# aanna0701/face-recognition-pytorch

Hardware: AMD Instinct MI355X
Metric: train imgs/sec IR-50-layout ResNet50 + ArcFace/PartialFC head, 112x112 (higher is better)
Workload: dtype bf16

## Files before the change

### face-recognition-pytorch_amd/frhip/csrc/igemm_nt.hip

```cpp
#include "igemm_nt.h"
#include "frhip.h"

namespace frhip {

bool halo_applicable(int dtype, int h, int w, int c, int k, int r, int s, int stride, int pad);
int halo_stat_rows(int dtype, int m, int w, int c, int k, int sign);
bool halo_xf_applicable(int dtype, int h, int w, int c, int k, int r, int s, int stride, int pad);
bool halo_lean_applies(int dtype, int n, int h, int w, int c, int k, int sign);
int halo_run(int dtype, const void* a, const void* b, void* out, const void* res, float* stats, const EpiBnRed& br,
             int n, int h, int w, int c, int k, int sign, hipStream_t stream, const float* xf_scale = nullptr,
             const float* xf_shift = nullptr, void* xf_out = nullptr);

enum { EPI_STORE = 0, EPI_ATOMIC = 1, EPI_SLAB = 2, EPI_LEAN = 3 };
extern int g_epi_lean;

template <typename T, int WM, int WN, int MT, int EPI>
__device__ __forceinline__ void nt_tile(const NtGeom& g, const void* __restrict__ a, const void* __restrict__ b, void* __restrict__ out,
                                        const void* __restrict__ res, float* __restrict__ stats, const EpiBnRed& br, int ntiles,
                                        uint32_t t, uint32_t total, char* smem) {
    typedef NtTile<T, WM, WN, MT> Tile;
    constexpr int WROWS = Tile::WROWS, THREADS = Tile::THREADS;
    const uint32_t lin = xcd_remap(t, total);
    const int ntile = (int)(lin % (uint32_t)ntiles), mtile = (int)(lin / (uint32_t)ntiles);
    const int ks_begin = blockIdx.y * g.ksteps_per_split;
    const int ks_end = min(g.ksteps, ks_begin + g.ksteps_per_split);

    NtMainloop<T, WM, WN, MT> ml;
    ml.run(g, a, b, smem, mtile, ntile, ks_begin, ks_end);

    const int lane = lane_id(), wave = wave_id();
    const int wm = wave / WN, wn = wave % WN;
    const int m0 = mtile * Tile::BM + wm * WROWS, n0 = ntile * Tile::BN + wn * 64;

    if constexpr (EPI == EPI_LEAN) {
        if (stats && br.y && !br.gelu_bwd) {
            constexpr int P = Tile::template stage_pitch<T>();
            float accs[2][4] = {{0.f, 0.f, 0.f, 0.f}, {0.f, 0.f, 0.f, 0.f}};
#pragma unroll
            for (int half = 0; half < 2; ++half) {
                EpiOperands<T, 64> eo;
                eo.fetch_fast(res, br.y, g.M, g.Nout, m0 + 64 * half, n0);
                const char* mine = ml.stage_half(smem, half);
                nt_epilogue_store_fast<T, WM, WN, 64, THREADS, Tile::BN>(mine, P, smem, g.M, g.Nout, out, res != nullptr, stats, br, eo, mtile, ntile,
                                                                         64 * P, accs);
            }
            epi_stats_tail_mfma<WM, WN, THREADS, Tile::BN>(accs[0], accs[1], smem, g.Nout, stats, mtile, ntile);
        } else {
            const char* mine = ml.template stage_out<T>(smem);
            nt_epilogue_store_lean<WM, WN, WROWS, THREADS, Tile::BN>(mine, Tile::template stage_pitch<T>(), smem, g.M, g.Nout, out, res, stats, br,
                                                                     mtile, ntile, m0, n0);
        }
    } else if constexpr (EPI == EPI_STORE) {
        EpiOperands<T, WROWS> eo;
        eo.fetch(res, (stats || br.gelu_bwd) ? br.y : nullptr, g.M, g.Nout, m0, n0, br.res_h, br.res_w, &br.map);
        const char* mine = ml.template stage_out<T>(smem);
        nt_epilogue_store<T, WM, WN, WROWS, THREADS, Tile::BN>(mine, Tile::template stage_pitch<T>(), smem, g.M, g.Nout, out,
                                                               res != nullptr, stats, br, eo, mtile, ntile, m0, n0);
    } else {
        constexpr int P = Tile::template stage_pitch<float>();
        const char* mine = ml.template stage_out<float>(smem);
        float* o = reinterpret_cast<float*>(out);
        const int n = n0 + lane;
        if constexpr (EPI == EPI_SLAB) o += (size_t)blockIdx.y * g.M * g.Nout;
        for (int row = 0; row < WROWS; ++row) {
            const int m = m0 + row;
            if (m < g.M && n < g.Nout) {
                const float v = *reinterpret_cast<const float*>(mine + row * P + lane * 4);
                if constexpr (EPI == EPI_SLAB) o[(size_t)m * g.Nout + n] = v;
                else atomicAdd(o + (size_t)m * g.Nout + n, v);
            }
        }
    }
}

template <typename T, int WM, int WN, int MT, int EPI>
__global__ __launch_bounds__(64 * WM * WN, (WM * WN) / 4) void nt_kernel(NtGeom g, const void* __restrict__ a,
                                                           const void* __restrict__ b, void* __restrict__ out,
                                                           const void* __restrict__ res, float* __restrict__ stats,
                                                           EpiBnRed br, int mtiles, int ntiles) {
    extern __shared__ __attribute__((aligned(16))) char smem[];
    const uint32_t total = (uint32_t)(mtiles * ntiles);
    if constexpr (EPI == EPI_LEAN) {
        for (uint32_t t = blockIdx.x; t < total; t += gridDim.x) {
            nt_tile<T, WM, WN, MT, EPI>(g, a, b, out, res, stats, br, ntiles, t, total, smem);
            if (t + gridDim.x < total) {
                asm volatile("s_waitcnt lgkmcnt(0)" ::: "memory");
                __builtin_amdgcn_s_barrier();
            }
        }
    } else {
        nt_tile<T, WM, WN, MT, EPI>(g, a, b, out, res, stats, br, ntiles, blockIdx.x, total, smem);
    }
}

template <typename T, int WM, int WN, int MT, int EPI>
static int nt_launch_cfg(const NtGeom& g, const void* a, const void* b, void* out, const void* res,
                         float* stats, const EpiBnRed& br, int splits, hipStream_t stream) {
    typedef NtTile<T, WM, WN, MT> Tile;
    const int mtiles = (g.M + Tile::BM - 1) / Tile::BM, ntiles = (g.Nout + Tile::BN - 1) / Tile::BN;
    const int lds = (EPI == EPI_STORE || EPI == EPI_LEAN) ? Tile::template lds_bytes<T>() : Tile::template lds_bytes<float>();
    auto kern = nt_kernel<T, WM, WN, MT, EPI>;
    if (set_dynamic_lds(reinterpret_cast<const void*>(kern), lds, "igemm_nt")) return FRHIP_ELAUNCH;
    dim3 grid(mtiles * ntiles, splits);
    if (EPI == EPI_LEAN) {
        const unsigned wgs = (unsigned)device_cu_count() & ~7u;
        if (wgs >= 8 && grid.x > wgs) grid.x = wgs;
    }
    hipLaunchKernelGGL(kern, grid, dim3(Tile::THREADS), lds, stream, g, a, b, out, res, stats, br, mtiles, ntiles);
    return check_launch("igemm_nt");
}

static int g_nt_tile = 0;

static int nt_pick_tile(int dtype, const NtGeom& g) {
    if (g_nt_tile) return (dtype != FRHIP_DT_BF16 && g_nt_tile >= 3) ? 1 : g_nt_tile;
    if ((g.Nout % 128) != 0 && g.Nout <= 256) return 2;
    if (dtype == FRHIP_DT_BF16 && (g.Nout % 256) == 0 && g.M >= 256 * 64) return 4;
    return 1;
}

static const EpiBnRed NO_BNRED = {nullptr, nullptr, nullptr, nullptr, nullptr, 0, 0, {0, 0, 0, 0, 0, 0}, nullptr, nullptr, 0};

static int nt_dispatch(int dtype, const NtGeom& g, const void* a, const void* b, void* out, const void* res,
                       float* stats, const EpiBnRed& br, int splits, bool atomic, hipStream_t stream) {
    const int tile = nt_pick_tile(dtype, g);
#define NT_GO(T, WM, WN, MT)                                                                              \
    return atomic ? nt_launch_cfg<T, WM, WN, MT, EPI_ATOMIC>(g, a, b, out, res, stats, br, splits, stream)     \
                  : nt_launch_cfg<T, WM, WN, MT, EPI_STORE>(g, a, b, out, res, stats, br, splits, stream)
    if (dtype == FRHIP_DT_BF16 && (tile == 3 || tile == 4)) {
        if (tile == 4 && !atomic && splits == 1 && g_epi_lean && nt_lean_ok(true, g.M, g.Nout, br, stats))
            return nt_launch_cfg<bf16_t, 2, 4, 8, EPI_LEAN>(g, a, b, out, res, stats, br, splits, stream);
        if (tile == 4 && !atomic) return nt_launch_cfg<bf16_t, 2, 4, 8, EPI_STORE>(g, a, b, out, res, stats, br, splits, stream);
        NT_GO(bf16_t, 4, 2, 4);
    }
    return by_dtype(dtype, "igemm_nt", [&](auto t) {
        typedef decltype(t) T;
        if (tile == 2) NT_GO(T, 4, 1, 4);
        NT_GO(T, 2, 2, 4);
    });
#undef NT_GO
}

static int esize(int dtype) { return dtype == FRHIP_DT_BF16 ? 2 : 4; }

static int fill_geom(NtGeom& g, int dtype, int n, int h, int w, int c, int ho, int wo, int k, int r, int s,
                     int stride, int pad, int mode, const char* who) {
    const int bke = NT_ROWB / esize(dtype);
    if (n <= 0 || h <= 0 || w <= 0 || c <= 0 || k <= 0 || (c % bke) != 0 || (k % 8) != 0 || (stride != 1 && stride != 2)) {
        set_error("%s: unsupported shape n=%d h=%d w=%d c=%d k=%d stride=%d (c must be a multiple of %d, k of 8)",
                  who, n, h, w, c, k, stride, bke);
        return FRHIP_EINVAL;
    }
    const long long a_bytes = 1LL * n * h * w * c * esize(dtype), b_bytes = 1LL * k * r * s * c * esize(dtype);
    if (a_bytes > 0x7fffffffLL || b_bytes > 0x7fffffffLL || 1LL * n * ho * wo > 0x7fffffffLL) {
        set_error("%s: tensor exceeds the 2 GiB buffer-addressing window", who);
        return FRHIP_EINVAL;
    }
    g.H = h; g.W = w; g.C = c; g.Ho = ho; g.Wo = wo; g.R = r; g.S = s; g.stride = stride; g.pad = pad; g.mode = mode;
    g.M = n * ho * wo; g.Nout = k; g.Ktot = r * s * c;
    g.ksteps = r * s * (c / bke); g.ksteps_per_split = g.ksteps;
    g.a_bytes = (uint32_t)a_bytes; g.b_bytes = (uint32_t)b_bytes;
    g.par_a = -1; g.par_b = -1; g.hc = 0; g.wc = 0; g.par_r0 = 0; g.par_s0 = 0;
    return FRHIP_OK;
}

static bool dgrad_by_parity(const NtGeom& g) { return g.mode == 1 && g.stride == 2 && g.R == 3 && g.S == 3 && g.pad == 1; }

static int nt_block_rows(int dtype, const NtGeom& g) {
    static const int bm_of[5] = {128, 128, 256, 256, 256};
    return bm_of[nt_pick_tile(dtype, g)];
}

static int parity_class(const NtGeom& g, int dtype, int a, int b, NtGeom& gc, OutMap& map) {
    gc = g;
    gc.par_a = a; gc.par_b = b;
    gc.hc = (g.Ho - a + 1) / 2; gc.wc = (g.Wo - b + 1) / 2;
    gc.par_r0 = (a + g.pad) & 1; gc.par_s0 = (b + g.pad) & 1;
    const int nr = (g.R - gc.par_r0 + 1) / 2, ns = (g.S - gc.par_s0 + 1) / 2;
    const int n_img = g.M / (g.Ho * g.Wo);
    gc.M = n_img * gc.hc * gc.wc;
    gc.ksteps = nr * ns * (g.C / (NT_ROWB / (dtype == FRHIP_DT_BF16 ? 2 : 4)));
    gc.ksteps_per_split = gc.ksteps;
    map.hc = gc.hc; map.wc = gc.wc; map.ho = g.Ho; map.wo = g.Wo; map.a = a; map.b = b;
    return gc.M;
}

}

using namespace frhip;

extern "C" int frhip_nt_block_m(int nout) {
    return ((nout % 128) == 0 || nout > 256) ? 128 : 256;
}
extern "C" int frhip_conv_stat_rows(int dtype, int m, int k, int h, int w, int c, int r, int s, int stride, int pad) {
    if (halo_applicable(dtype, h, w, c, k, r, s, stride, pad)) return halo_stat_rows(dtype, m, w, c, k, +1);
    NtGeom g; g.M = m; g.Nout = k;
    static const int bm_of[5] = {128, 128, 256, 256, 256};
    const int bm = bm_of[nt_pick_tile(dtype, g)];
    return (m + bm - 1) / bm;
}
extern "C" int frhip_set_nt_tile(int tile) { const int old = g_nt_tile; g_nt_tile = tile; return old; }

extern "C" int frhip_conv_fwd(int dtype, const void* x, const void* w, void* y, float* stats_partial,
                              int n, int h, int wd, int c, int k, int r, int s, int stride, int pad,
                              hipStream_t stream) {
    if (const int rc = by_dtype(dtype, "frhip_conv_fwd", [](auto) { return FRHIP_OK; })) return rc;
    NtGeom g;
    const int ho = (h + 2 * pad - r) / stride + 1, wo = (wd + 2 * pad - s) / stride + 1;
    int rc = fill_geom(g, dtype, n, h, wd, c, ho, wo, k, r, s, stride, pad, 0, "frhip_conv_fwd");
    if (rc) return rc;
    if (halo_applicable(dtype, h, wd, c, k, r, s, stride, pad))
        return halo_run(dtype, x, w, y, nullptr, stats_partial, NO_BNRED, n, h, wd, c, k, +1, stream);
    return nt_dispatch(dtype, g, x, w, y, nullptr, stats_partial, NO_BNRED, 1, false, stream);
}

extern "C" int frhip_conv_fwd_affine(int dtype, const void* x, const void* w, void* y, const float* scale, const float* shift, int relu,
                                     const void* residual, int n, int h, int wd, int c, int k, int r, int s, int stride, int pad,
                                     hipStream_t stream) {
    if (const int rc = by_dtype(dtype, "frhip_conv_fwd_affine", [](auto) { return FRHIP_OK; })) return rc;
    if (!scale || !shift) { set_error("frhip_conv_fwd_affine: scale and shift are required"); return FRHIP_EINVAL; }
    NtGeom g;
    const int ho = (h + 2 * pad - r) / stride + 1, wo = (wd + 2 * pad - s) / stride + 1;
    int rc = fill_geom(g, dtype, n, h, wd, c, ho, wo, k, r, s, stride, pad, 0, "frhip_conv_fwd_affine");
    if (rc) return rc;
    if (halo_applicable(dtype, h, wd, c, k, r, s, stride, pad) && halo_lean_applies(dtype, n, h, wd, c, k, +1)) {
        EpiBnRed br = NO_BNRED;
        br.aff_scale = scale; br.aff_shift = shift; br.aff_relu = relu;
        return halo_run(dtype, x, w, y, residual, nullptr, br, n, h, wd, c, k, +1, stream);
    }
    rc = frhip_conv_fwd(dtype, x, w, y, nullptr, n, h, wd, c, k, r, s, stride, pad, stream);
    if (rc) return rc;
    return frhip_bn_apply(dtype, y, scale, shift, residual, nullptr, nullptr, relu, y, n * ho * wo, k, stream);
}

extern "C" int frhip_conv_bnrelu_fusable(int dtype, int h, int wd, int c, int k, int r, int s, int stride, int pad) {
    return halo_xf_applicable(dtype, h, wd, c, k, r, s, stride, pad) ? 1 : 0;
}

extern "C" int frhip_conv_fwd_bnrelu(int dtype, const void* x, const float* in_scale, const float* in_shift, const void* w, void* y,
                                     float* stats_partial, void* act_out, int n, int h, int wd, int c, int k, int r, int s, int stride,
                                     int pad, hipStream_t stream) {
    if (const int rc = by_dtype(dtype, "frhip_conv_fwd_bnrelu", [](auto) { return FRHIP_OK; })) return rc;
    if (!in_scale || !in_shift || !halo_xf_applicable(dtype, h, wd, c, k, r, s, stride, pad)) {
        set_error("frhip_conv_fwd_bnrelu: not fusable for this shape (ask frhip_conv_bnrelu_fusable first)");
        return FRHIP_EINVAL;
    }
    return halo_run(dtype, x, w, y, nullptr, stats_partial, NO_BNRED, n, h, wd, c, k, +1, stream, in_scale, in_shift, act_out);
}

static int dgrad_run(int dtype, const void* dy, const void* wt, void* dx, const void* residual, float* stats,
                     const EpiBnRed& br, int n, int h, int wd, int c, int k, int r, int s, int stride, int pad,
                     hipStream_t stream, const char* who) {
    NtGeom g;
    const int ho = (h + 2 * pad - r) / stride + 1, wo = (wd + 2 * pad - s) / stride + 1;
    int rc = fill_geom(g, dtype, n, ho, wo, k, h, wd, c, r, s, stride, pad, 1, who);
    if (rc) return rc;
    if (halo_applicable(dtype, h, wd, k, c, r, s, stride, pad))
        return halo_run(dtype, dy, wt, dx, residual, stats, br, n, h, wd, k, c, -1, stream);
    if (dgrad_by_parity(g)) {
        float* st = stats;
        for (int cls = 0; cls < 4; ++cls) {
            NtGeom gc; EpiBnRed bc = br;
            if (parity_class(g, dtype, cls >> 1, cls & 1, gc, bc.map) == 0) continue;
            rc = nt_dispatch(dtype, gc, dy, wt, dx, residual, st, bc, 1, false, stream);
            if (rc) return rc;
            if (st) st += (size_t)((gc.M + nt_block_rows(dtype, gc) - 1) / nt_block_rows(dtype, gc)) * 2 * gc.Nout;
        }
        return FRHIP_OK;
    }
    return nt_dispatch(dtype, g, dy, wt, dx, residual, stats, br, 1, false, stream);
}

extern "C" int frhip_conv_dgrad(int dtype, const void* dy, const void* wt, void* dx, const void* residual,
                                int n, int h, int wd, int c, int k, int r, int s, int stride, int pad,
                                hipStream_t stream) {
    if (const int rc = by_dtype(dtype, "frhip_conv_dgrad", [](auto) { return FRHIP_OK; })) return rc;
    return dgrad_run(dtype, dy, wt, dx, residual, nullptr, NO_BNRED, n, h, wd, c, k, r, s, stride, pad, stream, "frhip_conv_dgrad");
}

extern "C" int frhip_dgrad_stat_rows(int dtype, int n, int h, int wd, int c, int k, int r, int s, int stride, int pad) {
    const int m = n * h * wd;
    if (halo_applicable(dtype, h, wd, k, c, r, s, stride, pad)) return halo_stat_rows(dtype, m, wd, k, c, -1);
    NtGeom g; g.M = m; g.Nout = c;
    g.mode = 1; g.stride = stride; g.R = r; g.S = s; g.pad = pad; g.Ho = h; g.Wo = wd; g.C = k;
    if (dgrad_by_parity(g)) {
        int rows = 0;
        for (int cls = 0; cls < 4; ++cls) {
            NtGeom gc; OutMap map;
            const int mc = parity_class(g, dtype, cls >> 1, cls & 1, gc, map);
            rows += (mc + nt_block_rows(dtype, gc) - 1) / nt_block_rows(dtype, gc);
        }
        return rows;
    }
    const int bm = nt_block_rows(dtype, g);
    return (m + bm - 1) / bm;
}

extern "C" int frhip_conv_dgrad_fused(int dtype, const void* dy, const void* wt, void* dx, const void* residual,
                                      int residual_stride, const void* y_bn, const float* mean, const float* invstd,
                                      const float* mask_scale, const float* mask_shift, float* stats_partial, int n, int h,
                                      int wd, int c, int k, int r, int s, int stride, int pad, hipStream_t stream) {
    if (const int rc = by_dtype(dtype, "frhip_conv_dgrad_fused", [](auto) { return FRHIP_OK; })) return rc;
    if (residual_stride != 1 && residual_stride != 2) { set_error("frhip_conv_dgrad_fused: residual_stride must be 1 or 2"); return FRHIP_EINVAL; }
    if (y_bn && (!mean || !invstd || !stats_partial || (mask_scale && !mask_shift))) {
        set_error("frhip_conv_dgrad_fused: y_bn needs mean, invstd and stats_partial");
        return FRHIP_EINVAL;
    }
    EpiBnRed br = {y_bn, mean, invstd, mask_scale, mask_shift, 0, 0, {0, 0, 0, 0, 0, 0}, nullptr, nullptr, 0};
    if (residual && residual_stride == 2) { br.res_h = h; br.res_w = wd; }
    return dgrad_run(dtype, dy, wt, dx, residual, y_bn ? stats_partial : nullptr, br, n, h, wd, c, k, r, s, stride, pad, stream,
                     "frhip_conv_dgrad_fused");
}

extern "C" int frhip_conv_dgrad_fused_rs(int dtype, const void* dy, const void* wt, void* dx, const void* residual,
                                         int residual_stride, const void* y_bn, const float* mean, const float* invstd,
                                         const float* mask_scale, const float* mask_shift, const float* rowscale, int rows_per,
                                         float keep_scale, float* stats_partial, int n, int h, int wd, int c, int k, int r, int s,
                                         int stride, int pad, hipStream_t stream) {
    if (const int rc = by_dtype(dtype, "frhip_conv_dgrad_fused_rs", [](auto) { return FRHIP_OK; })) return rc;
    if (residual_stride != 1 && residual_stride != 2) { set_error("frhip_conv_dgrad_fused_rs: residual_stride must be 1 or 2"); return FRHIP_EINVAL; }
    if (!y_bn || !mean || !invstd || !stats_partial || (mask_scale && !mask_shift) || !rowscale || rows_per <= 0 ||
        (long long)n * h * wd % rows_per != 0) {
        set_error("frhip_conv_dgrad_fused_rs: y_bn, mean, invstd, stats_partial, rowscale and a rows_per that divides the rows are required");
        return FRHIP_EINVAL;
    }
    EpiBnRed br = {y_bn, mean, invstd, mask_scale, mask_shift, 0, 0, {0, 0, 0, 0, 0, 0}, nullptr, nullptr, 0};
    br.rowkeep = rowscale; br.rows_per = rows_per; br.keep_scale = keep_scale;
    if (residual && residual_stride == 2) { br.res_h = h; br.res_w = wd; }
    return dgrad_run(dtype, dy, wt, dx, residual, stats_partial, br, n, h, wd, c, k, r, s, stride, pad, stream, "frhip_conv_dgrad_fused_rs");
}

extern "C" int frhip_conv_dgrad_bnred(int dtype, const void* dy, const void* wt, void* dx, const void* residual,
                                      const void* y_bn, const float* mean, const float* invstd, const float* mask_scale,
                                      const float* mask_shift, float* stats_partial, int n, int h, int wd, int c, int k,
                                      int r, int s, int stride, int pad, hipStream_t stream) {
    if (const int rc = by_dtype(dtype, "frhip_conv_dgrad_bnred", [](auto) { return FRHIP_OK; })) return rc;
    if (!y_bn || !mean || !invstd || !stats_partial || (mask_scale && !mask_shift)) {
        set_error("frhip_conv_dgrad_bnred: y_bn, mean, invstd and stats_partial are required");
        return FRHIP_EINVAL;
    }
    return frhip_conv_dgrad_fused(dtype, dy, wt, dx, residual, 1, y_bn, mean, invstd, mask_scale, mask_shift, stats_partial,
                                  n, h, wd, c, k, r, s, stride, pad, stream);
}

extern "C" int frhip_linear_fwd(int dtype, const void* a, const void* w, const float* bias, void* out, void* act_out,
                                float* stats_partial, int m, int n, int k, hipStream_t stream) {
    if (const int rc = by_dtype(dtype, "frhip_linear_fwd", [](auto) { return FRHIP_OK; })) return rc;
    NtGeom g;
    int rc = fill_geom(g, dtype, m, 1, 1, k, 1, 1, n, 1, 1, 1, 0, 0, "frhip_linear_fwd");
    if (rc) return rc;
    EpiBnRed br = NO_BNRED;
    br.bias = bias; br.act = act_out;
    return nt_dispatch(dtype, g, a, w, out, nullptr, stats_partial, br, 1, false, stream);
}

extern "C" int frhip_linear_dgrad_gelu(int dtype, const void* dy, const void* wt, const void* pre, void* dx,
                                       float* stats_partial, int m, int n, int k, hipStream_t stream) {
    if (const int rc = by_dtype(dtype, "frhip_linear_dgrad_gelu", [](auto) { return FRHIP_OK; })) return rc;
    if (!pre) { set_error("frhip_linear_dgrad_gelu: the saved pre-activation is required"); return FRHIP_EINVAL; }
    NtGeom g;
    int rc = fill_geom(g, dtype, m, 1, 1, k, 1, 1, n, 1, 1, 1, 0, 0, "frhip_linear_dgrad_gelu");
    if (rc) return rc;
    EpiBnRed br = NO_BNRED;
    br.y = pre; br.gelu_bwd = 1;
    return nt_dispatch(dtype, g, dy, wt, dx, nullptr, stats_partial, br, 1, false, stream);
}

namespace frhip {
__global__ __launch_bounds__(256) void nt_slab_reduce_kernel(const float* __restrict__ slabs, int splits, size_t elems,
                                                             const float* __restrict__ bias, int n, float* __restrict__ out) {
    const size_t i = ((size_t)blockIdx.x * 256 + threadIdx.x) * 4;
    if (i >= elems) return;
    f32x4_t acc = *reinterpret_cast<const f32x4_t*>(slabs + i);
    for (int s = 1; s < splits; ++s) acc += *reinterpret_cast<const f32x4_t*>(slabs + (size_t)s * elems + i);
    if (bias) acc += *reinterpret_cast<const f32x4_t*>(bias + (i % (size_t)n));
    *reinterpret_cast<f32x4_t*>(out + i) = acc;
}
}

extern "C" int frhip_gemm_nt_splitk(int dtype, const void* a, const void* b, const float* bias, float* out, int m, int n,
                                    int k, int splits, float* slabs, size_t slab_bytes, hipStream_t stream) {
    return by_dtype(dtype, "frhip_gemm_nt_splitk", [&](auto t) {
        NtGeom g;
        int rc = fill_geom(g, dtype, m, 1, 1, k, 1, 1, n, 1, 1, 1, 0, 0, "frhip_gemm_nt_splitk");
        if (rc) return rc;
        if (n % 4) { set_error("frhip_gemm_nt_splitk: n must be a multiple of 4"); return FRHIP_EINVAL; }
        if (splits < 1) splits = 1;
        if (splits > g.ksteps) splits = g.ksteps;
        g.ksteps_per_split = (g.ksteps + splits - 1) / splits;
        splits = (g.ksteps + g.ksteps_per_split - 1) / g.ksteps_per_split;
        const size_t elems = (size_t)m * n;
        if (!slabs || slab_bytes < elems * 4 * (size_t)splits) { set_error("frhip_gemm_nt_splitk: workspace too small (%zu bytes needed)", elems * 4 * (size_t)splits); return FRHIP_EINVAL; }
        rc = nt_launch_cfg<decltype(t), 2, 2, 4, EPI_SLAB>(g, a, b, slabs, nullptr, nullptr, NO_BNRED, splits, stream);
        if (rc) return rc;
        hipLaunchKernelGGL(nt_slab_reduce_kernel, dim3((unsigned)((elems / 4 + 255) / 256)), dim3(256), 0, stream, slabs, splits, elems, bias, n, out);
        return check_launch("frhip_gemm_nt_splitk/reduce");
    });
}

extern "C" int frhip_gemm_nt(int dtype, const void* a, const void* b, void* out, int m, int n, int k,
                             int splits, int atomic_f32, hipStream_t stream) {
    if (const int rc = by_dtype(dtype, "frhip_gemm_nt", [](auto) { return FRHIP_OK; })) return rc;
    NtGeom g;
    int rc = fill_geom(g, dtype, m, 1, 1, k, 1, 1, n, 1, 1, 1, 0, 0, "frhip_gemm_nt");
    if (rc) return rc;
    if (!atomic_f32 || splits < 1) splits = 1;
    if (splits > g.ksteps) splits = g.ksteps;
    g.ksteps_per_split = (g.ksteps + splits - 1) / splits;
    splits = (g.ksteps + g.ksteps_per_split - 1) / g.ksteps_per_split;
    return nt_dispatch(dtype, g, a, b, out, nullptr, nullptr, NO_BNRED, splits, atomic_f32 != 0, stream);
}
```

### include/frhip.h

```cpp
#ifndef FRHIP_H
#define FRHIP_H
#include <stddef.h>
#include <stdint.h>

#ifdef __cplusplus
extern "C" {
#endif

#ifndef FRHIP_STREAM_T
#define FRHIP_STREAM_T
#ifdef __HIP_PLATFORM_AMD__
#include <hip/hip_runtime_api.h>
typedef hipStream_t frhip_stream_t;
#else
typedef void* frhip_stream_t;
#endif
#endif

#define FRHIP_OK 0
#define FRHIP_EINVAL (-1)
#define FRHIP_ELAUNCH (-2)
#define FRHIP_DT_BF16 0
#define FRHIP_DT_F32 1

const char* frhip_last_error(void);
int frhip_abi_version(void);
int frhip_spin(long long ticks, frhip_stream_t stream);

int frhip_nt_block_m(int k);
int frhip_conv_stat_rows(int dtype, int m, int k, int h, int w, int c, int r, int s, int stride, int pad);
int frhip_set_wgrad_taps9(int enabled);
int frhip_set_conv_halo(int enabled);
int frhip_set_halo_wide_dirs(int dirs);
int frhip_set_epi_lean(int enabled);
int frhip_set_ew_batch(int enabled);
int frhip_set_nt_tile(int tile);
int frhip_conv_fwd_affine(int dtype, const void* x, const void* w, void* y, const float* scale, const float* shift, int relu,
                          const void* residual, int n, int h, int wd, int c, int k, int r, int s, int stride, int pad,
                          frhip_stream_t stream);
int frhip_conv_fwd(int dtype, const void* x, const void* w, void* y, float* stats_partial,
                   int n, int h, int wd, int c, int k, int r, int s, int stride, int pad, frhip_stream_t stream);
int frhip_conv_dgrad(int dtype, const void* dy, const void* wt, void* dx, const void* residual,
                     int n, int h, int wd, int c, int k, int r, int s, int stride, int pad, frhip_stream_t stream);
int frhip_dgrad_stat_rows(int dtype, int n, int h, int wd, int c, int k, int r, int s, int stride, int pad);
int frhip_conv_dgrad_bnred(int dtype, const void* dy, const void* wt, void* dx, const void* residual,
                           const void* y_bn, const float* mean, const float* invstd, const float* mask_scale,
                           const float* mask_shift, float* stats_partial, int n, int h, int wd, int c, int k,
                           int r, int s, int stride, int pad, frhip_stream_t stream);
int frhip_conv_dgrad_fused(int dtype, const void* dy, const void* wt, void* dx, const void* residual, int residual_stride,
                           const void* y_bn, const float* mean, const float* invstd, const float* mask_scale,
                           const float* mask_shift, float* stats_partial, int n, int h, int wd, int c, int k,
                           int r, int s, int stride, int pad, frhip_stream_t stream);
int frhip_conv_dgrad_fused_rs(int dtype, const void* dy, const void* wt, void* dx, const void* residual, int residual_stride,
                              const void* y_bn, const float* mean, const float* invstd, const float* mask_scale,
                              const float* mask_shift, const float* rowscale, int rows_per, float keep_scale,
                              float* stats_partial, int n, int h, int wd, int c, int k, int r, int s, int stride, int pad,
                              frhip_stream_t stream);
int frhip_conv_wgrad(int dtype, const void* dy, const void* x, float* dw, int n, int h, int w, int c,
                     int k, int r, int s, int stride, int pad, int splits, float* workspace, size_t workspace_bytes,
                     frhip_stream_t stream);
int frhip_conv_wgrad_chain_ok(int dtype, int n, int h, int w, int c, int k, int r, int s, int stride, int pad);
int frhip_conv_wgrad_chain(int dtype, const void* dy, const void* x, int n, int h, int w, int c, int k, float* slabs,
                           size_t slab_bytes, float* prev_dw, const float* prev_slabs, int prev_k, int prev_c, int prev_splits,
                           int* splits_out, frhip_stream_t stream);
int frhip_conv_wgrad_chain_finish(float* dw, float* slabs, int k, int c, int splits, frhip_stream_t stream);
int frhip_wgrad_plan(int dtype, int n, int h, int w, int c, int kc, int ldp, int r, int s, int stride, int pad, int splits,
                     int have_workspace, size_t workspace_bytes, int overwrite, int transform, int* plan_out);
int frhip_linear_fwd(int dtype, const void* a, const void* w, const float* bias, void* out, void* act_out,
                     float* stats_partial, int m, int n, int k, frhip_stream_t stream);
int frhip_linear_dgrad_gelu(int dtype, const void* dy, const void* wt, const void* pre, void* dx, float* stats_partial,
                            int m, int n, int k, frhip_stream_t stream);
int frhip_gemm_nt(int dtype, const void* a, const void* b, void* out, int m, int n, int k, int splits,
                  int atomic_f32, frhip_stream_t stream);
int frhip_gemm_nt_splitk(int dtype, const void* a, const void* b, const float* bias, float* out, int m, int n, int k,
                         int splits, float* slabs, size_t slab_bytes, frhip_stream_t stream);
int frhip_gemm_tn(int dtype, const void* p, const void* q, float* out, int m, int kc, int ldp, int c,
                  int splits, float* workspace, size_t workspace_bytes, frhip_stream_t stream);
int frhip_gemm_tn_overwrite(int dtype, const void* p, const void* q, float* out, int m, int kc, int ldp, int c,
                            float* workspace, size_t workspace_bytes, frhip_stream_t stream);

int frhip_colreduce_blocks(int rows, int c, int dtype);
int frhip_colstats(int dtype, const void* x, int rows, int c, float* partial, frhip_stream_t stream);
int frhip_bn_finalize(const float* partial, int nparts, float* scratch, int c, float count,
                      const float* gamma, const float* beta, float* running_mean, float* running_var,
                      float momentum, float eps, float* mean, float* invstd, float* scale, float* shift,
                      frhip_stream_t stream);
int frhip_bn_eval_affine(int c, const float* gamma, const float* beta, const float* running_mean,
                         const float* running_var, float eps, float* scale, float* shift, frhip_stream_t stream);
int frhip_bn_standin_state(int c, const float* gamma, const float* beta, float k, float* mean, float* invstd, float* scale,
                           float* shift, frhip_stream_t stream);
int frhip_bn_apply(int dtype, const void* y, const float* scale, const float* shift, const void* res,
                   const float* res_scale, const float* res_shift, int relu, void* out, int rows, int c,
                   frhip_stream_t stream);
int frhip_bn_bwd_reduce(int dtype, const void* dout, const void* y, const float* mean, const float* invstd,
                        const float* mask_scale, const float* mask_shift, int rows, int c, float* partial,
                        frhip_stream_t stream);
int frhip_bn_bwd_finalize(const float* partial, int nparts, float* scratch, int c, float count,
                          const float* gamma, const float* mean, const float* invstd, float* dgamma,
                          float* dbeta, float* ca, float* cb, float* cc, frhip_stream_t stream);
int frhip_bn_eval_state(int c, const float* gamma, const float* beta, const float* running_mean, const float* running_var, float eps,
                        float* mean, float* invstd, float* scale, float* shift, frhip_stream_t stream);
int frhip_bn_bwd_finalize_eval(const float* partial, int nparts, float* scratch, int c, float count,
                               const float* gamma, const float* mean, const float* invstd, float* dgamma,
                               float* dbeta, float* ca, float* cb, float* cc, frhip_stream_t stream);
int frhip_bn_bwd_apply(int dtype, const void* dout, const void* y, const float* ca, const float* cb,
                       const float* cc, const float* mask_scale, const float* mask_shift, void* dy,
                       int rows, int c, frhip_stream_t stream);
int frhip_bn_apply_rs(int dtype, const void* y, const float* scale, const float* shift, const void* res, const float* rowscale,
                      int rows_per, void* out, int rows, int c, frhip_stream_t stream);
int frhip_bn_bwd_reduce_rs(int dtype, const void* dout, const void* y, const float* mean, const float* invstd, const float* rowscale,
                           int rows_per, int rows, int c, float* partial, frhip_stream_t stream);
int frhip_bn_bwd_apply_rs(int dtype, const void* dout, const void* y, const float* ca, const float* cb, const float* cc,
                          const float* rowscale, int rows_per, void* dy, int rows, int c, frhip_stream_t stream);
int frhip_sum_partials(const float* partial, int nparts, int c, int which, float* out_accum, frhip_stream_t stream);
int frhip_add_bias(float* x, const float* bias, int rows, int c, frhip_stream_t stream);
int frhip_cast_from_f32(int dtype, const float* src, void* dst, size_t n, frhip_stream_t stream);
int frhip_cast_to_f32(int dtype, const void* src, float* dst, size_t n, frhip_stream_t stream);

int frhip_stem_im2col(int dtype, const float* x, void* col, int b, int h, int w, int stride, frhip_stream_t stream);
int frhip_bn_relu_maxpool_fwd(int dtype, const void* y, const float* scale, const float* shift, void* out,
                              uint8_t* argmax, int b, int h, int w, int c, frhip_stream_t stream);
int frhip_maxpool_bwd(int dtype, const void* dpool, const uint8_t* argmax, void* da, int b, int h, int w,
                      int c, frhip_stream_t stream);

int frhip_pack_wt(int dtype, const float* w, void* wt, int k, int rs, int c, frhip_stream_t stream);
int frhip_transpose2d(int dtype_in, int dtype_out, const void* in, void* out, int rows, int cols, int ld_out,
                      frhip_stream_t stream);
int frhip_pack_stem(int dtype, const float* w, void* wp, int k, int kin, int kp, frhip_stream_t stream);
int frhip_unpack_stem_grad(const float* dwp, float* dw, int k, int kin, int kp, frhip_stream_t stream);
int frhip_fc_permute(int dtype, const float* w, void* wp, int nout, int c, int hw, frhip_stream_t stream);
int frhip_fc_unpermute_grad(const float* dwp, float* dw, int nout, int c, int hw, frhip_stream_t stream);
int frhip_pfc_sample_max_local(void);
int frhip_pfc_sample(const int64_t* labels, int n, long long class_start, int num_local, const float* u, int num_sample,
                     int64_t* index_out, int* rel_out, int64_t* n_positive, frhip_stream_t stream);
int frhip_gather_rows(const float* src, const int64_t* index, float* dst, int n, int d, frhip_stream_t stream);
int frhip_scatter_rows(const float* src, const int64_t* index, float* dst, int n, int d, frhip_stream_t stream);

int frhip_head_dw_ok(int dtype, int n, int classes, int d);
int frhip_head_dw(int dtype, const void* dt, int ldt, const void* ehat, const void* what, const float* wnorm, float* dw,
                  int n, int classes, int d, float out_scale, frhip_stream_t stream);
int frhip_l2norm_rows(int dtype, const float* x, void* xhat, float* norms, int rows, int d, float eps,
                      frhip_stream_t stream);
int frhip_l2norm_bwd(int dtype, const float* dxhat, const void* xhat, const float* norms, float* dx,
                     int rows, int d, float out_scale, frhip_stream_t stream);
int frhip_l2norm_bwd_norm(int dtype, const float* dxhat, const void* xhat, const float* norms, const float* dnorm, float* dx,
                          int rows, int d, float out_scale, frhip_stream_t stream);
int frhip_head_groups(int num_classes);
int frhip_head_fwd(int dtype, const void* ehat, const void* what, const int* labels, int n, int classes,
                   int d, float s, float m, float* part_max, float* part_sum, float* ztarget,
                   float* rowmax, float* rowsum, frhip_stream_t stream);
int frhip_head_rescale(float* rowsum, const float* local_max, const float* global_max, int n, frhip_stream_t stream);
int frhip_head_target_prob(const float* ztarget, const int* labels, const float* rowmax, const float* rowsum,
                           float* q, int n, frhip_stream_t stream);
int frhip_head_pack_stats(const float* ztarget, const int* labels, const float* rowmax, const float* rowsum,
                          float* packed, int n, frhip_stream_t stream);
int frhip_head_merge_stats(const float* gathered, int world_size, int n, float* rowmax, float* rowsum, float* q,
                           frhip_stream_t stream);
int frhip_head_loss(const float* q, int n, float* loss, frhip_stream_t stream);
int frhip_head_bwd_dt(int dtype, const void* ehat, const void* what, const int* labels, int n, int classes,
                      int d, float s, float m, const float* rowmax, const float* rowsum, float gscale,
                      const float* upstream, void* dt, int ldt, void* dtt, int ldtt, frhip_stream_t stream);

#define FRHIP_MARGIN_ARCFACE 0
#define FRHIP_MARGIN_COSFACE 1
typedef struct { int kind; int easy; float s, m, filter_thr; } frhip_margin_t;
int frhip_head_fwd_ex(int dtype, const void* ehat, const void* what, const int* labels, int n, int classes,
                      int d, const frhip_margin_t* margin, float* part_max, float* part_sum, float* ztarget,
                      float* rowmax, float* rowsum, frhip_stream_t stream);
int frhip_head_bwd_dt_ex(int dtype, const void* ehat, const void* what, const int* labels, int n, int classes,
                         int d, const frhip_margin_t* margin, const float* rowmax, const float* rowsum, float gscale,
                         const float* upstream, void* dt, int ldt, void* dtt, int ldtt, frhip_stream_t stream);

typedef struct { float s, eps; const float* m_ang; const float* m_add; } frhip_margin_rows_t;
int frhip_adaface_margins(const float* norms, int n, double m, double h, double t_alpha, double eps, int update, float* batch_mean,
                          float* batch_std, float* m_ang, float* m_add, frhip_stream_t stream);
int frhip_magface_margins(const float* norms, int n, double l_a, double u_a, double l_m, double u_m, float* m_ang, float* m_add,
                          float* reg, frhip_stream_t stream);
int frhip_magface_norm_grad(const float* norms, const float* packed, int world_size, int n, const float* rowmax, const float* rowsum,
                            float s, float eps, double l_a, double u_a, double l_m, double u_m, double lambda_g, double gscale,
                            const float* upstream, double out_scale, float* dnorm, frhip_stream_t stream);
int frhip_head_fwd_rows(int dtype, const void* ehat, const void* what, const int* labels, int n, int classes,
                        int d, const frhip_margin_rows_t* margin, float* part_max, float* part_sum, float* ztarget,
                        float* rowmax, float* rowsum, frhip_stream_t stream);
int frhip_head_bwd_dt_rows(int dtype, const void* ehat, const void* what, const int* labels, int n, int classes,
                           int d, const frhip_margin_rows_t* margin, const float* rowmax, const float* rowsum, float gscale,
                           const float* upstream, void* dt, int ldt, void* dtt, int ldtt, frhip_stream_t stream);

int frhip_head_sub_max(void);
int frhip_head_fwd_sub(int dtype, const void* ehat, const void* what, const int* labels, int n, int classes, int d,
                       int subcenters, const frhip_margin_t* margin, float* part_max, float* part_sum, float* ztarget,
                       int* tsub, float* rowmax, float* rowsum, frhip_stream_t stream);
int frhip_head_fwd_sub_rows(int dtype, const void* ehat, const void* what, const int* labels, int n, int classes, int d,
                            int subcenters, const frhip_margin_rows_t* margin, float* part_max, float* part_sum,
                            float* ztarget, int* tsub, float* rowmax, float* rowsum, frhip_stream_t stream);
int frhip_head_bwd_dt_sub(int dtype, const void* ehat, const void* what, const int* labels, int n, int classes, int d,
                          int subcenters, const frhip_margin_t* margin, const float* rowmax, const float* rowsum,
                          float gscale, const float* upstream, void* dt, int ldt, int ldp, void* dtt, int ldtt,
                          frhip_stream_t stream);
int frhip_head_bwd_dt_sub_rows(int dtype, const void* ehat, const void* what, const int* labels, int n, int classes, int d,
                               int subcenters, const frhip_margin_rows_t* margin, const float* rowmax, const float* rowsum,
                               float gscale, const float* upstream, void* dt, int ldt, int ldp, void* dtt, int ldtt,
                               frhip_stream_t stream);

int frhip_conv_bnrelu_fusable(int dtype, int h, int wd, int c, int k, int r, int s, int stride, int pad);
int frhip_conv_fwd_bnrelu(int dtype, const void* x, const float* in_scale, const float* in_shift, const void* w, void* y,
                          float* stats_partial, void* act_out, int n, int h, int wd, int c, int k, int r, int s, int stride,
                          int pad, frhip_stream_t stream);
int frhip_conv_wgrad_bnrelu_fusable(int dtype, int n, int h, int w, int c, int k, int r, int s, int stride, int pad);
int frhip_conv_wgrad_bnrelu(int dtype, const void* dy, const void* x, const float* in_scale, const float* in_shift,
                            float* dw, int n, int h, int w, int c, int k, int r, int s, int stride, int pad, int splits,
                            float* workspace, size_t workspace_bytes, frhip_stream_t stream);

int frhip_quant_fp8_weights(const float* w, void* w8, float* scale, int k, int rowlen, frhip_stream_t stream);
typedef struct { const float* w; void* w8; float* scale; int32_t k, rowlen, row_begin, pad_; } frhip_q8w;
int frhip_quant_fp8_weights_multi(const frhip_q8w* table, int ntensors, int nrows, frhip_stream_t stream);
int frhip_fp8_saturation(int op);
int frhip_quant_fp8(int dtype, const void* x, void* x8, size_t n, float inv_scale, frhip_stream_t stream);
int frhip_bn_apply_q8(int dtype, const void* y, const float* scale, const float* shift, const void* res,
                      const float* res_scale, const float* res_shift, int relu, void* out, void* out8, float inv_q,
                      int rows, int c, frhip_stream_t stream);
int frhip_conv_fwd_fp8(const void* x8, const void* w8, const float* wscale, float act_scale, void* y,
                       float* stats_partial, int n, int h, int wd, int c, int k, int r, int s, int stride, int pad,
                       frhip_stream_t stream);
int frhip_fp8_stat_rows(int m, int k);
int frhip_fp8_conv_stat_rows(int m, int k, int h, int w, int c, int r, int s, int stride, int pad);
int frhip_set_fp8_halo(int enabled);
int frhip_linear_fwd_fp8(const void* a8, const void* w8, const float* wscale, float act_scale, const float* bias,
                         void* out, float* stats_partial, int m, int n, int k, frhip_stream_t stream);

typedef struct frhip_cpb_block {
    const void* coords;
    const void* index;
    const void* w0;
    const void* b0;
    const void* w2;
    const void* logit_scale;
    void* bias;
    void* scale;
    const void* dbias;
    const void* dscale;
    void* dw0;
    void* db0;
    void* dw2;
    void* dlogit_scale;
    int entries, tokens, heads, pad_;
} frhip_cpb_block;
int frhip_cpb_limits(int* max_entries, int* max_heads, int* hidden);
int frhip_cpb_scratch_floats(int nblocks);
int frhip_cpb_fwd(const frhip_cpb_block* blocks_dev, int nblocks, float* scratch, frhip_stream_t stream);
int frhip_cpb_bwd(const frhip_cpb_block* blocks_dev, int nblocks, float* scratch, frhip_stream_t stream);

int frhip_margin_fwd(float* logits, const int64_t* labels, int n, int c, float s, float m, int kind, float* tsave,
                     frhip_stream_t stream);
int frhip_margin_bwd(const float* gout, const int64_t* labels, const float* tsave, int n, int c, float s, float m,
                     int kind, float* gin, frhip_stream_t stream);
int frhip_margin_fwd_ex(float* logits, const int64_t* labels, int n, int c, const frhip_margin_t* margin, float* tsave,
                        uint64_t* filtered, frhip_stream_t stream);
int frhip_margin_bwd_ex(const float* gout, const int64_t* labels, const float* tsave, const uint64_t* filtered, int n, int c,
                        const frhip_margin_t* margin, float* gin, frhip_stream_t stream);
int frhip_margin_fwd_rows(const float* logits, const int64_t* labels, int n, int c, const frhip_margin_rows_t* margin, float* out,
                          frhip_stream_t stream);
int frhip_margin_bwd_rows(const float* gout, const float* logits, const int64_t* labels, int n, int c,
                          const frhip_margin_rows_t* margin, float* gin, frhip_stream_t stream);
int frhip_rows_max(const float* x, int n, int c, float* rowmax, frhip_stream_t stream);
int frhip_rows_exp_sum(float* x, int n, int c, const float* rowmax, float* rowsum, frhip_stream_t stream);
int frhip_rows_normalize(float* x, int n, int c, const float* rowsum, const int64_t* labels, float* ptarget,
                         frhip_stream_t stream);
int frhip_ce_grad(float* p, int n, int c, const int64_t* labels, float inv_n, const float* upstream,
                  frhip_stream_t stream);

int frhip_winattn_fwd(int dtype, const void* qkv, const float* bias, const float* scale, void* out, int b, int h,
                      int w, int c, int heads, int ws, int shift, frhip_stream_t stream);
int frhip_winattn_bwd(int dtype, const void* qkv, const void* dout, const float* bias, const float* scale,
                      void* dqkv, float* dbias, float* dscale, int b, int h, int w, int c, int heads,
                      int ws, int shift, float* workspace, size_t workspace_bytes, frhip_stream_t stream);
int frhip_winattn_bwd_colsum(int dtype, const void* qkv, const void* dout, const float* bias, const float* scale,
                             void* dqkv, float* dbias, float* dscale, float* dqkv_colsum, int b, int h, int w, int c,
                             int heads, int ws, int shift, float* workspace, size_t workspace_bytes, frhip_stream_t stream);
int frhip_winattn_bwd_qvbias(int dtype, const void* qkv, const void* dout, const float* bias, const float* scale,
                             void* dqkv, float* dbias, float* dscale, float* dq_bias, float* dv_bias, int b, int h, int w,
                             int c, int heads, int ws, int shift, float* workspace, size_t workspace_bytes, frhip_stream_t stream);
int frhip_set_winattn_mfma(int enabled);
int frhip_bias_gelu_fwd(int dtype, void* y, const float* bias, void* act_out, int rows, int c, frhip_stream_t stream);
int frhip_gelu_bwd(int dtype, const void* da, const void* h, void* dh, size_t n, frhip_stream_t stream);

int frhip_pair_score(const float* e1, const float* e2, const int64_t* labels, int n, int d, double* scores,
                     int* hist_idx, int* hist_genuine, int* hist_imposter, frhip_stream_t stream);
int frhip_cross_score(const float* e, const int64_t* labels, int n, int d, double* scores, double* pair_labels,
                      int* hist_idx, int* hist_genuine, int* hist_imposter, frhip_stream_t stream);
int frhip_cross_hist(const float* e, const int64_t* labels, int64_t n, int d, int64_t i0, int64_t i1, uint64_t* hist_genuine,
                     uint64_t* hist_imposter, uint64_t* thr_genuine, uint64_t* thr_imposter, frhip_stream_t stream);
int frhip_gallery_topk(const float* probe, const float* gallery, const int64_t* exclude, int64_t p, int64_t g, int d, int k,
                       int64_t g0, int64_t g1, double* top_score, int64_t* top_index, void* workspace, size_t workspace_bytes,
                       frhip_stream_t stream);
int frhip_gallery_topk_workspace(int64_t p, int k, int64_t* bytes);

int frhip_stem_blocks(int b, int h, int w);
int frhip_set_stem_scatter(int enabled);
int frhip_stem_stats(int dtype, const float* x, const void* wp, int b, int h, int w, float* partial, frhip_stream_t stream);
int frhip_stem_fwd(int dtype, const float* x, const void* wp, const float* scale, const float* shift, void* pooled,
                   uint8_t* argmax, int b, int h, int w, frhip_stream_t stream);
int frhip_stem_bwd_reduce(int dtype, const float* x, const void* wp, const void* dpool, const uint8_t* argmax,
                          const float* mean, const float* invstd, const float* scale, const float* shift, int b, int h,
                          int w, float* partial, frhip_stream_t stream);
int frhip_stem_bwd_wgrad(int dtype, const float* x, const void* wp, const void* dpool, const uint8_t* argmax,
                         const float* ca, const float* cb, const float* cc, const float* scale, const float* shift, int b,
                         int h, int w, float* slabs, float* dw, frhip_stream_t stream);
int frhip_stem_gram_floats(void);
int frhip_stem_gram_blocks(int b, int h, int w);
int frhip_stem_gram(int dtype, const float* x, int b, int h, int w, float* partial, float* gram, frhip_stream_t stream);
int frhip_stem_bwd_wgrad_gram(int dtype, const float* x, const void* wp, const void* dpool, const void* pooled,
                              const uint8_t* argmax, const float* gram, const float* ca, const float* cb, const float* cc,
                              int b, int h, int w, float* slabs, float* dw, frhip_stream_t stream);
int frhip_stem_dx(int dtype, const float* x, const void* wp, const void* dpool, const uint8_t* argmax, const void* pooled,
                  const float* ca, const float* cb, const float* cc, int b, int h, int w, float* dx, frhip_stream_t stream);
int frhip_stem_dx_s2(int dtype, const void* dy0, const void* wp, int kp, int b, int h, int w, float* dx, frhip_stream_t stream);

typedef struct { const float* w; void* wc; void* wt; int32_t k, rs, c, tile_begin; } frhip_wprep;
int frhip_prep_conv_weights(int dtype, const frhip_wprep* table, int ntensors, int ntiles, frhip_stream_t stream);

int frhip_dropout_mask(int dtype, void* mask, size_t n, float keep, long long seed, frhip_stream_t stream);

int frhip_augment_u8(const uint8_t* in, float* out, const int32_t* flip, const int32_t* holes, int nholes,
                     int b, int hin, int win, int size, frhip_stream_t stream);
int frhip_augment_u8_lut(const uint8_t* in, const uint8_t* lut, float* out, const int32_t* flip, const int32_t* holes,
                         int nholes, int b, int hin, int win, int size, frhip_stream_t stream);
int frhip_motion_blur_u8(const uint8_t* in, uint8_t* out, const uint8_t* lut, const float* kernels, const int32_t* ksize,
                         int b, int h, int w, frhip_stream_t stream);
int frhip_iso_noise_scratch_doubles(int b);
int frhip_iso_noise_u8(const uint8_t* in, uint8_t* out, double* scratch, const float* params, const int32_t* lum_noise,
                       const float* color_noise, const uint64_t* seeds, int b, int h, int w, frhip_stream_t stream);

#define FRHIP_SGD_CHUNK 65536
#define FRHIP_SGD_MAX_GROUPS 8
typedef struct { float lr, weight_decay, momentum, clip; } frhip_sgd_group;
typedef struct { float* p; const float* g; float* m; uint32_t n; uint32_t group; } frhip_sgd_chunk;
int frhip_sgd_clip_coef(const frhip_sgd_chunk* chunks, int nchunks, const frhip_sgd_group* groups_host, int ngroups,
                        float max_norm, float* partial, float* coef_out, frhip_stream_t stream);
int frhip_sgd_multi(const frhip_sgd_chunk* chunks, int nchunks, const frhip_sgd_group* groups_host, int ngroups,
                    const float* clip_coef, frhip_stream_t stream);

typedef struct { float lr, beta1, beta2, eps, weight_decay, bc1, bc2, clip; } frhip_adamw_group;
typedef struct { float* p; const float* g; float* m; float* v; uint32_t n; uint32_t group; } frhip_adamw_chunk;
int frhip_adamw_clip_coef(const frhip_adamw_chunk* chunks, int nchunks, const frhip_adamw_group* groups_host, int ngroups,
                          float max_norm, float* partial, float* coef_out, frhip_stream_t stream);
int frhip_adamw_multi(const frhip_adamw_chunk* chunks, int nchunks, const frhip_adamw_group* groups_host, int ngroups,
                      const float* clip_coef, frhip_stream_t stream);

#ifdef __cplusplus
}
#endif
#endif
```

Baseline: 22740.

## Merge stride-2 dgrad parity-class GEMMs into one launch ordered by tap count

For stride-2 3x3 dgrad split into four output-parity classes, it now launches a single kernel covering all classes whenever they share one tile config. Each block finds its class from a prefix table of block offsets. Classes are ordered by descending tap count so the heaviest work starts first. This removes three extra kernel launches and the tail idle time between sequential small launches, at the cost of a slightly larger kernel argument block and per-block class lookup.

Result: no change. 22800, median of 6 (+0.3%).

```diff
diff --git a/face-recognition-pytorch_amd/frhip/csrc/igemm_nt.hip b/face-recognition-pytorch_amd/frhip/csrc/igemm_nt.hip
--- a/face-recognition-pytorch_amd/frhip/csrc/igemm_nt.hip
+++ b/face-recognition-pytorch_amd/frhip/csrc/igemm_nt.hip
@@ -1,4 +1,5 @@
 #include "igemm_nt.h"
+#include "nt_parity_plan.h"
 #include "frhip.h"
 
 namespace frhip {
@@ -93,6 +94,36 @@
     }
 }
 
+struct NtParityArgs {
+    NtGeom g[4];
+    OutMap map[4];
+    float* stats[4];
+    int first[5];
+};
+
+template <typename T, int WM, int WN, int MT>
+__global__ __launch_bounds__(64 * WM * WN, (WM * WN) / 4) void nt_parity_kernel(NtParityArgs p, const void* __restrict__ a,
+                                                                  const void* __restrict__ b, void* __restrict__ out,
+                                                                  const void* __restrict__ res, EpiBnRed br, int ntiles) {
+    extern __shared__ __attribute__((aligned(16))) char smem[];
+    const int bx = (int)blockIdx.x;
+    const int s = (bx >= p.first[1]) + (bx >= p.first[2]) + (bx >= p.first[3]);
+    br.map = p.map[s];
+    nt_tile<T, WM, WN, MT, EPI_STORE>(p.g[s], a, b, out, res, p.stats[s], br, ntiles, (uint32_t)(bx - p.first[s]),
+                                      (uint32_t)(p.first[s + 1] - p.first[s]), smem);
+}
+
+template <typename T, int WM, int WN, int MT>
+static int nt_parity_launch_cfg(const NtParityArgs& p, const void* a, const void* b, void* out, const void* res, const EpiBnRed& br,
+                                int ntiles, hipStream_t stream) {
+    typedef NtTile<T, WM, WN, MT> Tile;
+    const int lds = Tile::template lds_bytes<T>();
+    auto kern = nt_parity_kernel<T, WM, WN, MT>;
+    if (set_dynamic_lds(reinterpret_cast<const void*>(kern), lds, "igemm_nt")) return FRHIP_ELAUNCH;
+    hipLaunchKernelGGL(kern, dim3(p.first[4]), dim3(Tile::THREADS), lds, stream, p, a, b, out, res, br, ntiles);
+    return check_launch("igemm_nt");
+}
+
 template <typename T, int WM, int WN, int MT, int EPI>
 static int nt_launch_cfg(const NtGeom& g, const void* a, const void* b, void* out, const void* res,
                          float* stats, const EpiBnRed& br, int splits, hipStream_t stream) {
@@ -141,6 +172,17 @@
 #undef NT_GO
 }
 
+static int nt_parity_dispatch(int dtype, int tile, const NtParityArgs& p, const void* a, const void* b, void* out, const void* res,
+                              const EpiBnRed& br, int ntiles, hipStream_t stream) {
+    if (dtype == FRHIP_DT_BF16 && tile == 4) return nt_parity_launch_cfg<bf16_t, 2, 4, 8>(p, a, b, out, res, br, ntiles, stream);
+    if (dtype == FRHIP_DT_BF16 && tile == 3) return nt_parity_launch_cfg<bf16_t, 4, 2, 4>(p, a, b, out, res, br, ntiles, stream);
+    return by_dtype(dtype, "igemm_nt", [&](auto t) {
+        typedef decltype(t) T;
+        if (tile == 2) return nt_parity_launch_cfg<T, 4, 1, 4>(p, a, b, out, res, br, ntiles, stream);
+        return nt_parity_launch_cfg<T, 2, 2, 4>(p, a, b, out, res, br, ntiles, stream);
+    });
+}
+
 static int esize(int dtype) { return dtype == FRHIP_DT_BF16 ? 2 : 4; }
 
 static int fill_geom(NtGeom& g, int dtype, int n, int h, int w, int c, int ho, int wo, int k, int r, int s,
@@ -185,6 +227,22 @@
     return gc.M;
 }
 
+static int g_parity_merge = 1;
+
+static_assert(NT_PLAN_BM[1] == NtTile<bf16_t, 2, 2>::BM && NT_PLAN_BN[1] == NtTile<bf16_t, 2, 2>::BN &&
+              NT_PLAN_BM[2] == NtTile<bf16_t, 4, 1>::BM && NT_PLAN_BN[2] == NtTile<bf16_t, 4, 1>::BN &&
+              NT_PLAN_BM[3] == NtTile<bf16_t, 4, 2>::BM && NT_PLAN_BN[3] == NtTile<bf16_t, 4, 2>::BN &&
+              NT_PLAN_BM[4] == NtTile<bf16_t, 2, 4, 8>::BM && NT_PLAN_BN[4] == NtTile<bf16_t, 2, 4, 8>::BN,
+              "nt_parity_plan.h plans for the tiles of this file");
+
+static NtParityPlan parity_plan(const NtGeom& g, int dtype) {
+    return nt_parity_plan(g.M / (g.Ho * g.Wo), g.Ho, g.Wo, g.Nout, [&](int rows) {
+        NtGeom gc = g;
+        gc.M = rows;
+        return nt_pick_tile(dtype, gc);
+    });
+}
+
 }
 
 using namespace frhip;
@@ -258,6 +316,18 @@
     if (halo_applicable(dtype, h, wd, k, c, r, s, stride, pad))
         return halo_run(dtype, dy, wt, dx, residual, stats, br, n, h, wd, k, c, -1, stream);
     if (dgrad_by_parity(g)) {
+        const NtParityPlan pl = parity_plan(g, dtype);
+        if (g_parity_merge && pl.one_tile && pl.nonempty > 1) {
+            NtParityArgs p;
+            for (int slot = 0; slot < 4; ++slot) {
+                const NtParityClass& pc = pl.cls[pl.order[slot]];
+                parity_class(g, dtype, pc.a, pc.b, p.g[slot], p.map[slot]);
+                p.stats[slot] = stats ? stats + (size_t)pc.first_stat_row * 2 * g.Nout : nullptr;
+                p.first[slot] = pc.first_block;
+            }
+            p.first[4] = pl.blocks;
+            return nt_parity_dispatch(dtype, pl.tile, p, dy, wt, dx, residual, br, pl.col_tiles, stream);
+        }
         float* st = stats;
         for (int cls = 0; cls < 4; ++cls) {
             NtGeom gc; EpiBnRed bc = br;
@@ -294,6 +364,26 @@
     }
     const int bm = nt_block_rows(dtype, g);
     return (m + bm - 1) / bm;
+}
+
+extern "C" int frhip_set_dgrad_parity_merge(int enabled) { const int old = g_parity_merge; g_parity_merge = enabled; return old; }
+
+extern "C" int frhip_dgrad_parity_plan(int dtype, int n, int h, int wd, int c, int k, int* plan_out) {
+    if (const int rc = by_dtype(dtype, "frhip_dgrad_parity_plan", [](auto) { return FRHIP_OK; })) return rc;
+    NtGeom g;
+    const int ho = (h + 2 - 3) / 2 + 1, wo = (wd + 2 - 3) / 2 + 1;
+    if (const int rc = fill_geom(g, dtype, n, ho, wo, k, h, wd, c, 3, 3, 2, 1, 1, "frhip_dgrad_parity_plan")) return rc;
+    if (!plan_out) { set_error("frhip_dgrad_parity_plan: plan_out required"); return FRHIP_EINVAL; }
+    const NtParityPlan pl = parity_plan(g, dtype);
+    plan_out[0] = (g_parity_merge && pl.one_tile && pl.nonempty > 1) ? 1 : pl.nonempty;
+    plan_out[1] = pl.blocks; plan_out[2] = pl.stat_rows; plan_out[3] = pl.col_tiles;
+    for (int cls = 0; cls < 4; ++cls) {
+        const NtParityClass& kc = pl.cls[cls];
+        const int fields[8] = {kc.rows, kc.taps, kc.tile, kc.row_tiles, kc.blocks, kc.first_block, kc.first_stat_row, 0};
+        for (int i = 0; i < 8; ++i) plan_out[4 + 8 * cls + i] = fields[i];
+    }
+    for (int slot = 0; slot < 4; ++slot) plan_out[4 + 8 * pl.order[slot] + 7] = slot;
+    return FRHIP_OK;
 }
 
 extern "C" int frhip_conv_dgrad_fused(int dtype, const void* dy, const void* wt, void* dx, const void* residual,
diff --git a/face-recognition-pytorch_amd/frhip/csrc/nt_parity_plan.h b/face-recognition-pytorch_amd/frhip/csrc/nt_parity_plan.h
--- /dev/null
+++ b/face-recognition-pytorch_amd/frhip/csrc/nt_parity_plan.h
@@ -0,0 +1,60 @@
+#pragma once
+
+namespace frhip {
+
+constexpr int NT_PLAN_BM[5] = {128, 128, 256, 256, 256};
+constexpr int NT_PLAN_BN[5] = {128, 128, 64, 128, 256};
+
+struct NtParityClass {
+    int a, b, hc, wc;
+    int rows, taps;
+    int tile;
+    int row_tiles;
+    int blocks;
+    int first_block;
+    int first_stat_row;
+};
+
+struct NtParityPlan {
+    NtParityClass cls[4];
+    int order[4];
+    int tile, col_tiles;
+    int blocks, stat_rows;
+    int nonempty;
+    bool one_tile;
+};
+
+template <typename TileOf>
+inline NtParityPlan nt_parity_plan(int images, int ho, int wo, int nout, TileOf&& tile_of) {
+    NtParityPlan pl{};
+    pl.one_tile = true;
+    for (int c = 0; c < 4; ++c) {
+        NtParityClass& k = pl.cls[c];
+        k.a = c >> 1; k.b = c & 1;
+        k.hc = (ho - k.a + 1) / 2; k.wc = (wo - k.b + 1) / 2;
+        k.rows = images * k.hc * k.wc;
+        k.taps = (k.a ? 2 : 1) * (k.b ? 2 : 1);
+        if (k.rows > 0) {
+            k.tile = tile_of(k.rows);
+            const int bm = NT_PLAN_BM[k.tile], bn = NT_PLAN_BN[k.tile];
+            k.row_tiles = (k.rows + bm - 1) / bm;
+            k.blocks = k.row_tiles * ((nout + bn - 1) / bn);
+            pl.col_tiles = (nout + bn - 1) / bn;
+            if (pl.tile && pl.tile != k.tile) pl.one_tile = false;
+            pl.tile = k.tile;
+            ++pl.nonempty;
+        }
+        k.first_stat_row = pl.stat_rows;
+        pl.stat_rows += k.row_tiles;
+    }
+    static const int by_taps[4] = {3, 1, 2, 0};
+    for (int s = 0; s < 4; ++s) {
+        NtParityClass& k = pl.cls[by_taps[s]];
+        pl.order[s] = by_taps[s];
+        k.first_block = pl.blocks;
+        pl.blocks += k.blocks;
+    }
+    return pl;
+}
+
+}
diff --git a/include/frhip.h b/include/frhip.h
--- a/include/frhip.h
+++ b/include/frhip.h
@@ -51,6 +51,8 @@
                            const void* y_bn, const float* mean, const float* invstd, const float* mask_scale,
                            const float* mask_shift, float* stats_partial, int n, int h, int wd, int c, int k,
                            int r, int s, int stride, int pad, frhip_stream_t stream);
+int frhip_set_dgrad_parity_merge(int enabled);
+int frhip_dgrad_parity_plan(int dtype, int n, int h, int wd, int c, int k, int* plan_out);
 int frhip_conv_dgrad_fused_rs(int dtype, const void* dy, const void* wt, void* dx, const void* residual, int residual_stride,
                               const void* y_bn, const float* mean, const float* invstd, const float* mask_scale,
                               const float* mask_shift, const float* rowscale, int rows_per, float keep_scale,
```
